# drnatebrown/col-bwt

Hardware: AMD Instinct MI355X
Metric: query bases/s (higher is better)
Workload: dtype int64

## Files before the change

col-bwt_amd/csrc/fat2_query.hip:

```cpp
#include <hip/hip_runtime.h>
#include <stdint.h>

#include "device_layout.h"
#include "fat_cursor.h"
#include "fat_layout.h"
#include "lane_io.h"
#include "lane_out.h"
#include "query_kernels.h"

namespace colbwt {

namespace {

constexpr uint32_t kOffMis0 = 0xFFFFFFFCu;
constexpr uint32_t kOffMis1 = 0xFFFFFFFBu;

#ifdef COLBWT_COUNT_TRIPS
#define FAT2_STAT(k) (++stat[k])
__device__ unsigned long long g_fat2_more[2];
#else
#define FAT2_STAT(k) ((void)0)
#endif

__device__ __forceinline__ uint32_t mis_slot(const uint8_t *top, uint32_t own, uint32_t c) {
    const uint32_t aidx = top[own], cidx = top[c];
    const uint32_t slot = cidx < aidx ? cidx : cidx - 1;
    return cidx < 4 && slot < kFatSlots ? slot : kFatSlots;
}

template <int K, typename PmlT, bool kDeep>
__global__ __launch_bounds__(kQueryBlock)
void fat2_query_kernel(FatTable T, const uint8_t *__restrict__ bases, const uint64_t *__restrict__ read_off,
                       uint64_t n_reads, uint32_t big_reads, uint32_t tail_permille,
                       PmlT *__restrict__ pml, uint8_t *__restrict__ cid) {
    constexpr bool kWide = sizeof(PmlT) == 4;
    constexpr bool kTail = K == 8 && !kWide;
    __shared__ uint4 s_stage[kWaves][8][64];
    __shared__ uint4 s_win[kWaves][4][64];
    __shared__ uint32_t s_claim;
    __shared__ uint8_t s_top[256];
    __shared__ uint32_t s_tch[kTail ? 256 : 1];
    const uint32_t wave = threadIdx.x >> 6, lane = threadIdx.x & 63u, g8 = lane & ~7u, p = lane & 7u;
    uint32_t *const s_jx = reinterpret_cast<uint32_t *>(&s_stage[wave][7][48]);
    ChunkPlan plan;
    plan.init(n_reads, big_reads, tail_permille);
    if (threadIdx.x == 0) s_claim = 0;
    s_top[threadIdx.x] = (uint8_t)fat_top_index(T.top4, threadIdx.x);
    if constexpr (kTail) {
        const uint32_t b = threadIdx.x;
        s_tch[b] = ((T.top4 >> (8 * (b & 3u))) & 0xFFu) | (((T.top4 >> (8 * ((b >> 2) & 3u))) & 0xFFu) << 8) |
                   (((T.top4 >> (8 * ((b >> 4) & 3u))) & 0xFFu) << 16) | (((T.top4 >> (8 * (b >> 6))) & 0xFFu) << 24);
    }
    __syncthreads();
    uint32_t *const claim = &s_claim;
    ReadCursor rc;
    bool done;
    rc.c_next = threadIdx.x;
    rc.request_chunk(plan, read_off);
    rc.commit();
    done = !rc.enter_chunk(plan, claim);

    OutRuns acc;
    uint32_t trip = 0;
    LaneWindow win;
    win.init(rc.off + rc.k - 1);
    uint4 (*const my_win)[64] = s_win[wave];

    uint32_t j = done ? 0u : T.r - 1;
    uint32_t o = kOffLastPos;
    uint32_t L = 0;
    const uint4 *const my_row = &s_stage[wave][p][g8];

#ifdef COLBWT_COUNT_TRIPS
    unsigned long long stat[8] = {0, 0, 0, 0, 0, 0, 0, 0}, stat_full = 0, stat_hop15 = 0;
#endif
    while (__any(!done)) {
        bool step_back = false;
        if (!done && rc.k == 0 && !rc.next_in_flight && (rc.r != rc.r_lo || rc.nc_ready)) {
            if (rc.r != rc.r_lo) {
                rc.r -= 1;
                rc.k = rc.off - rc.next_off;
                rc.off = rc.next_off;
                step_back = rc.r > rc.r_lo;
            } else if (kWide || acc.cnt == 0) {
                done = !rc.enter_chunk(plan, claim);
                if (!done) win.init(rc.off + rc.k - 1);
            }
            j = done ? 0u : T.r - 1;
            o = kOffLastPos;
            L = 0;
        }
        const bool live = !done && rc.k != 0;
        uint64_t &k = rc.k;
        const uint64_t g = rc.off + k - 1;

        s_jx[lane] = j;
        wave_sync();
        {
            const uint4 ja = *reinterpret_cast<const uint4 *>(&s_jx[g8]);
            const uint4 jb = *reinterpret_cast<const uint4 *>(&s_jx[g8 + 4]);
            const uint32_t jq[8] = {ja.x, ja.y, ja.z, ja.w, jb.x, jb.y, jb.z, jb.w};
            wave_sync();
#pragma unroll
            for (uint32_t q = 0; q < 8; ++q)
                __builtin_amdgcn_global_load_lds(T.lines + (uint64_t)jq[q] * kFatRowBytes + ((p ^ q) << 4), &s_stage[wave][q][0],
                                                 16, 0, 0);
        }
        uint32_t want = 8u;
        if constexpr (kTail) want = T.match_tail && L >= 8u && o != kOffMis0 && o != kOffMis1 ? 16u : 8u;
        if (live && win.avail(g) < (k < want ? (uint32_t)k : want)) win.request(my_win, bases, g);
        if (step_back) { rc.in_next = read_off[rc.r - 1]; rc.next_in_flight = true; }
        if (!done && rc.fetch_pending) rc.request_chunk(plan, read_off);
        lds_dma_landed();
        rc.commit();

        const uint32_t have = live ? win.avail(g) : 0u;
        uint32_t consumed = 0, l_new = 0, keep = 0xFFFFFFFFu, keep1 = 0xFFFFFFFFu;
        uint64_t ids = 0, ids2 = 0;
        if (!live || have == 0) FAT2_STAT(5);
        if (live && have != 0) {
            const uint64_t W = win.get8(my_win, lane, g);
            const uint32_t left = k < have ? (uint32_t)k : have;
            if (o == kOffMis0 || o == kOffMis1) {
                FAT2_STAT(2);
                const uint32_t h4 = !kDeep && o == kOffMis1 ? 4u : 0u;
                const uint4 e0 = my_row[(h4 + 0u) ^ p], e1 = my_row[(h4 + 1u) ^ p], e2 = my_row[(h4 + 2u) ^ p],
                            e3 = my_row[(h4 + 3u) ^ p];
                const uint32_t carry = L;
                const uint32_t t1 = (e0.y >> 16) & 0xFFu, d1 = e0.y >> 24, v1 = e3.z & 7u;
                uint32_t oc = 4;
                if (left >= 2) {
                    const uint32_t c2 = (uint32_t)(W >> 48) & 0xFFu;
                    const uint32_t s2 = mis_slot(s_top, t1, c2);
                    if (c2 == t1) oc = 0;
                    else if (s2 < kFatSlots && ((v1 >> s2) & 1u)) oc = 1 + s2;
                }
                if (oc < 4) {
                    const uint32_t J = oc == 0 ? e0.z : oc == 1 ? e0.w : oc == 2 ? e1.x : e1.y;
                    const uint32_t rho = oc == 0 ? e1.z : oc == 1 ? e1.w : oc == 2 ? e2.x : e2.y;
                    const uint32_t pw = oc < 2 ? e2.z : e2.w, P = (oc & 1u) ? pw >> 16 : pw & 0xFFFFu;
                    const uint32_t ch = (e3.x >> (8 * oc)) & 0xFFu, cd = (e3.y >> (8 * oc)) & 0xFFu;
                    const uint32_t vo = (e3.z >> (4 + 4 * oc)) & 7u;
                    consumed = 2;
                    l_new = 1;
                    keep = oc == 0 ? 0xFFFFFFFFu : 0u;
                    ids = (uint64_t)(d1 | (carry << 8));
                    L = oc == 0 ? 1u : 0u;
                    uint32_t nJ = J, nP = P, nrho = rho, nch = ch, ncd = cd, nv = vo, seen = 2;
                    if constexpr (kDeep) {
                        if (left >= 3 && ((uint32_t)(W >> 40) & 0xFFu) == ch) {
                            const uint4 f0 = my_row[4u ^ p], f1 = my_row[5u ^ p], f2 = my_row[6u ^ p], f3 = my_row[7u ^ p];
                            nJ = oc == 0 ? f0.x : oc == 1 ? f0.y : oc == 2 ? f0.z : f0.w;
                            nrho = oc == 0 ? f1.x : oc == 1 ? f1.y : oc == 2 ? f1.z : f1.w;
                            const uint32_t pw2 = oc < 2 ? f2.x : f2.y;
                            nP = (oc & 1u) ? pw2 >> 16 : pw2 & 0xFFFFu;
                            nch = (f2.z >> (8 * oc)) & 0xFFu;
                            ncd = (f2.w >> (8 * oc)) & 0xFFu;
                            nv = (f3.x >> (4 * oc)) & 7u;
                            consumed = 3;
                            seen = 3;
                            ids = (uint64_t)(cd | (d1 << 8) | (carry << 16));
                            if (oc == 0) { l_new = 2; keep = 0xFFFFFFFFu; }
                            else { l_new = 1; keep = 0xFFFFFFFFu; keep1 = 0u; }
                            L += 1;
                        }
                    }
                    if (k > consumed) {
                        uint32_t sn = kFatSlots;
                        if (left > seen) {
                            const uint32_t cn = (uint32_t)(W >> (8u * (7u - seen))) & 0xFFu;
                            if (cn != nch) sn = mis_slot(s_top, nch, cn);
                        }
                        if (sn < kFatSlots && ((nv >> sn) & 1u)) {
                            const uint32_t e = nrho * kFatSlots + sn;
                            j = T.slot_line0 + (kDeep ? e : e >> 1);
                            o = kDeep ? kOffMis0 : kOffMis0 - (e & 1u);
                            L = ncd;
                        } else {
                            j = nJ;
                            o = nP;
                        }
                    }
                } else {
                    consumed = 1;
                    l_new = 0;
                    ids = (uint64_t)carry;
                    L = 0;
                    j = e0.x;
                    o = e0.y & 0xFFFFu;
                }
            } else {
                FAT2_STAT(0);
                const uint4 r0 = my_row[0 ^ p];
                const uint4 r1 = my_row[1 ^ p];
                const uint64_t CH = (uint64_t)r0.x | ((uint64_t)r0.y << 32);
                const uint64_t CID = (uint64_t)r0.z | ((uint64_t)r0.w << 32);
                const uint32_t len = r1.x & 0xFFFFu;
                uint32_t skip = 0;
                bool stay = false;
                if (o == kOffPred) { o = len - 1; skip = 1; }
                else if (o == kOffSucc) { o = 0; skip = 1; }
                else if (o >= len && j < T.r - 1) {
                    o -= len;
                    j += 1;
                    stay = true;
                    FAT2_STAT(1);
                } else {
                    o = o < len ? o : len - 1;
                }
                if (!stay) {
                    const uint64_t X = skip ? ((W >> 8) ^ CH) & 0x00FFFFFFFFFFFFFFull : W ^ CH;
                    const uint32_t run = matching_top_bytes(X);
                    const uint32_t cap = left + skip < (uint32_t)K ? left + skip : (uint32_t)K;
                    uint32_t steps = run < cap ? run : cap;
                    bool own_jump = true, to_entry = false;
                    uint32_t e_next = 0, carry = 0;
                    bool hop = false;
                    uint4 tl = make_uint4(0u, 0u, 0u, 0u);
                    if constexpr (kTail) {
                        if (T.match_tail && run == 8u && left + skip >= 16u && o < (r1.x >> 24) &&
                            acc.cnt + 16u + 8u * (3u - (trip & 3u)) <= 96u) {
                            tl = my_row[7 ^ p];
                            const uint64_t W2 = win.get8(my_win, lane, g - (8u - skip));
                            const uint64_t TC = (uint64_t)s_tch[(tl.w >> 16) & 0xFFu] | ((uint64_t)s_tch[tl.w >> 24] << 32);
                            hop = W2 == TC;
                        }
                    }
#ifdef COLBWT_COUNT_TRIPS
                    if (K == 8 && run == 8u && cap == 8u) ++stat_full;
#endif
                    if (run < cap) {
                        const uint32_t d = run + 1u, sh = 8u * (8u - d);
                        const uint32_t c = (uint32_t)(W >> (sh + 8u * skip)) & 0xFFu;
                        const uint32_t s = mis_slot(s_top, (uint32_t)(CH >> sh) & 0xFFu, c);
                        if (s < kFatSlots && ((r1.w >> (3u * run + s)) & 1u)) {
                            const uint32_t rho = reinterpret_cast<const uint32_t *>(&my_row[((kFatRho / 16) + (run >> 2)) ^ p])[run & 3u];
                            e_next = rho * kFatSlots + s;
                            carry = (uint32_t)(CID >> sh) & 0xFFu;
                            to_entry = true;
                            own_jump = false;
                        }
                    }
                    if (run == 0 && !to_entry) {
                        const uint32_t c = (uint32_t)(W >> 56);
                        const uint32_t cidx = T.cmap[c];
                        bool moved = false;
                        if (cidx != kAbsent) moved = fat_threshold_scan(T, j, o, c, cidx);
                        FAT2_STAT(moved ? 3 : 4);
                        if (moved) {
                            steps = 1;
                            consumed = 1;
                            l_new = 0;
                            own_jump = false;
                        } else {
                            const uint32_t st = matching_top_bytes(X & 0x00FFFFFFFFFFFFFFull);
                            const uint32_t cap0 = left < (uint32_t)K ? left : (uint32_t)K;
                            steps = st < cap0 ? st : cap0;
                            consumed = steps;
                            l_new = steps - 1;
                        }
                    } else {
                        consumed = (hop ? 16u : steps) - skip;
                        l_new = L + consumed;
                    }
                    L = l_new;
                    ids = steps ? CID >> (8u * (8u - steps)) : 0ull;
                    if (hop) {
                        FAT2_STAT(7);
#ifdef COLBWT_COUNT_TRIPS
                        stat_hop15 += skip;
#endif
                        ids2 = ids;
                        ids = (uint64_t)tl.x | ((uint64_t)tl.y << 32);
                    }
                    if (k == consumed) {
                    } else if (hop) {
                        j = tl.z;
                        o += tl.w & 0xFFFFu;
                    } else if (to_entry) {
                        FAT2_STAT(6);
                        j = T.slot_line0 + (kDeep ? e_next : e_next >> 1);
                        o = kDeep ? kOffMis0 : kOffMis0 - (e_next & 1u);
                        L = carry;
                    } else if (own_jump) {
                        const uint32_t e = steps - 1;
                        const uint32_t I = reinterpret_cast<const uint32_t *>(&my_row[((kFatI / 16) + (e >> 2)) ^ p])[e & 3u];
                        const uint32_t Oh = reinterpret_cast<const uint16_t *>(&my_row[((kFatO / 16) + (e >> 3)) ^ p])[e & 7u];
                        const uint64_t cuts = (uint64_t)r1.y | ((uint64_t)r1.z << 32);
                        const uint32_t cut = (uint32_t)(cuts >> (8 * e)) & 0xFFu, cut_a = cut & 0xFu, len_b = cut >> 4;
                        j = I;
                        if (cut_a != kSKCutNone && o >= cut_a) {
                            j += 1;
                            o -= cut_a;
                            if (len_b != kSKCutNone && o >= len_b) {
                                j += 1;
                                o -= len_b;
                            }
                        } else {
                            o += Oh;
                        }
                    }
                }
            }
            if constexpr (kWide) {
                for (uint32_t e = 0; e < consumed; ++e) {
                    pml[g - consumed + 1 + e] = (PmlT)((e < 2 ? keep : keep1) ? l_new - e : 0u);
                    cid[g - consumed + 1 + e] = (uint8_t)(ids >> (8 * e));
                }
            } else {
                if constexpr (kTail) acc.template push_run<true>(consumed, l_new, keep, keep1, (uint32_t)ids, (uint32_t)(ids >> 32), (uint32_t)ids2, (uint32_t)(ids2 >> 32));
                else acc.push_run(consumed, l_new, keep, keep1, (uint32_t)ids, (uint32_t)(ids >> 32));
            }
            k -= consumed;
        }
        wave_sync();
        if constexpr (!kWide) {
#ifdef COLBWT_ABL_NO_FLUSH
            if ((trip & (OutRuns::kPeriod - 1)) == OutRuns::kPeriod - 1) acc.cnt = acc.cnt > 90 ? 1 : 0;
#else
            if ((trip & (OutRuns::kPeriod - 1)) == OutRuns::kPeriod - 1)
                acc.flush_wave((uint16_t *)pml, cid, rc.off + rc.k, !done, rc.k == 0 && rc.r == rc.r_lo, &s_stage[wave][0][0], lane);
#endif
        }
        ++trip;
        wave_sync();
    }
#ifdef COLBWT_COUNT_TRIPS
    for (int q = 0; q < 8; ++q) atomicAdd(&g_fat_stats[q], stat[q]);
    atomicAdd(&g_fat2_more[0], stat_full);
    atomicAdd(&g_fat2_more[1], stat_hop15);
#endif
}

template <int K>
void launch_steps2(const FatTable &T, const uint8_t *d_bases, const uint64_t *d_read_off, uint64_t n_reads, uint64_t n_bases,
                   void *d_pml, int pml_bytes, uint8_t *d_cid, hipStream_t stream) {
    const bool deep = T.entry_shift == 7;
    if (pml_bytes == 2 && deep) launch_persistent<fat2_query_kernel<K, uint16_t, true>>(T, d_bases, d_read_off, n_reads, n_bases, (uint16_t *)d_pml, d_cid, stream);
    else if (pml_bytes == 2) launch_persistent<fat2_query_kernel<K, uint16_t, false>>(T, d_bases, d_read_off, n_reads, n_bases, (uint16_t *)d_pml, d_cid, stream);
    else if (deep) launch_persistent<fat2_query_kernel<K, uint32_t, true>>(T, d_bases, d_read_off, n_reads, n_bases, (uint32_t *)d_pml, d_cid, stream);
    else launch_persistent<fat2_query_kernel<K, uint32_t, false>>(T, d_bases, d_read_off, n_reads, n_bases, (uint32_t *)d_pml, d_cid, stream);
}

}

void launch_fat2_query(const FatTable &T, const uint8_t *d_bases, const uint64_t *d_read_off, uint64_t n_reads, uint64_t n_bases,
                       void *d_pml, int pml_bytes, uint8_t *d_cid, hipStream_t stream) {
    if (n_reads == 0) return;
#define X(K) \
    if (T.steps == K) launch_steps2<K>(T, d_bases, d_read_off, n_reads, n_bases, d_pml, pml_bytes, d_cid, stream);
    COLBWT_FAT_STEPS(X)
#undef X
}

#ifdef COLBWT_COUNT_TRIPS
extern "C" int colbwt_debug_fat2_stats(unsigned long long *out10, int reset) {
    if (hipMemcpyFromSymbol(out10, HIP_SYMBOL(g_fat_stats), 8 * sizeof(unsigned long long)) != hipSuccess) return -1;
    if (hipMemcpyFromSymbol(out10 + 8, HIP_SYMBOL(g_fat2_more), 2 * sizeof(unsigned long long)) != hipSuccess) return -1;
    if (reset) {
        unsigned long long z[8] = {0, 0, 0, 0, 0, 0, 0, 0};
        if (hipMemcpyToSymbol(HIP_SYMBOL(g_fat_stats), z, sizeof(z)) != hipSuccess) return -1;
        if (hipMemcpyToSymbol(HIP_SYMBOL(g_fat2_more), z, 2 * sizeof(unsigned long long)) != hipSuccess) return -1;
    }
    return 0;
}
#endif

}
```

col-bwt_amd/csrc/fat_build.hip:

```cpp
#include <hip/hip_runtime.h>
#include <stdint.h>

#include <functional>
#include <string>
#include <vector>

#include "../../include/colbwt.h"
#include "dev_mem.h"
#include "device_layout.h"
#include "fat_layout.h"
#include "jump_tables.h"
#include "lf_device.h"
#include "query_kernels.h"
#include "read_sampler.h"
#include "refine.h"

namespace colbwt {

namespace {

struct PlainLevel {
    const uint64_t *idx;
    const uint32_t *I;
    const uint16_t *O;
// ... 218 lines not shown
        }
        put_byte(w, kFatCut + (s - 1), cut | (len_b << 4));
    }

    if constexpr (kMis && K == 8) {
        uint64_t span = len < kFatTSpanMax ? len : kFatTSpanMax;
        uint32_t tch = 0;
        for (uint32_t a = 1; a <= kFatTailSteps + 1; ++a) {
            const uint64_t jl = P.idx[(uint64_t)j + 1] - P.idx[j];
            const uint64_t room = t < jl ? jl - t : 0;
            span = span < room ? span : room;
            if (a > kFatTailSteps) break;
            const uint32_t meta = P.meta[j];
            const uint32_t x = fat_top_index(T.top4, meta & 0xFFu);
            if (x >= 4) span = 0;
            tch |= (x & 3u) << (2 * (8 - a));
            put_byte(w, kFatTCid + (8 - a), meta >> 8);
            plain_lf(P, j, t);
        }
        if (span != 0) {
            put_half(w, kFatTCh, tch);
            w[kFatTI / 4] = j;
            put_half(w, kFatTO, (uint32_t)t);
            put_byte(w, kFatTSpan, (uint32_t)span);
            atomicAdd(tail_rows, 1ull);
        } else {
            w[kFatTCid / 4] = 0;
            w[kFatTCid / 4 + 1] = 0;
        }
    }
    if constexpr (kMis) {
        put_byte(w, kFatFlags, sflags[i]);
    } else {
        const uint32_t a_dense = T.cmap[own_ch];
        const uint32_t aidx = a_dense < 4 ? a_dense : kFatOwnOther;
        uint32_t flags = aidx << 4;
        const uint32_t top = T.sigma < 4 ? T.sigma : 4;
        for (uint32_t cidx = 0; cidx < top; ++cidx) {
            if (cidx == a_dense) continue;
            const uint32_t slot = hint_slot(cidx, a_dense);
            if (slot >= kFatSlots) continue;
            uint32_t tj;
            uint64_t to;
            if (!fat_slot_target(P, T, i, cidx, tj, to)) continue;
            flags |= 1u << slot;
            const uint32_t sb = kFatSlot0 + slot * kFatSlotBytes;
            plain_lf(P, tj, to);
            w[sb >> 2] = tj;
            put_half(w, sb + kFatSlotP, (uint32_t)to);
            const uint32_t meta = P.meta[tj];
            put_byte(w, sb + kFatSlotCh2, meta & 0xFFu);
            put_byte(w, sb + kFatSlotCid2, meta >> 8);
            plain_lf(P, tj, to);
            w[(sb >> 2) + 1] = tj;
            put_half(w, sb + kFatSlotP + 2, (uint32_t)to);
        }
        put_byte(w, kFatFlags, flags);
    }
    uint4 *dst = reinterpret_cast<uint4 *>(lines + (uint64_t)i * kFatRowBytes);
#pragma unroll
    for (uint32_t q = 0; q < kFatRowBytes / 16; ++q) dst[q] = make_uint4(w[4 * q], w[4 * q + 1], w[4 * q + 2], w[4 * q + 3]);
}

template <bool kDeep>
__global__ __launch_bounds__(256) void fat_mis_pack_kernel(PlainLevel P, FatTable T, const uint32_t *__restrict__ rho,
                                                           const uint32_t *__restrict__ rho_first,
                                                           const uint8_t *__restrict__ sflags, uint8_t *__restrict__ entries) {
    const uint64_t e = (uint64_t)blockIdx.x * 256 + threadIdx.x;
    if (e >= (uint64_t)T.n_rho * kFatSlots) return;
    constexpr uint32_t kDwords = (kDeep ? 2 * kMisBytes : kMisBytes) / 4;
    uint32_t w[kDwords];
#pragma unroll
    for (uint32_t q = 0; q < kDwords; ++q) w[q] = 0;
    const uint32_t i = rho_first[e / kFatSlots], slot = (uint32_t)(e % kFatSlots);
    if ((sflags[i] >> slot) & 1u) {
        const uint32_t a_dense = T.cmap[P.meta[i] & 0xFFu];
        uint32_t tj;
        uint64_t to;
        fat_slot_target(P, T, i, slot < a_dense ? slot : slot + 1, tj, to);
        plain_lf(P, tj, to);
        const uint32_t J1 = tj;
        const uint64_t P1 = to;
        const uint32_t m1 = P.meta[J1], a1 = T.cmap[m1 & 0xFFu], v1 = sflags[J1] & 7u;
        w[kMisJ1] = J1;
        w[kMisP1] = (uint32_t)P1 | ((m1 & 0xFFu) << 16) | ((m1 >> 8) << 24);
        w[kMisVal] = v1;
        for (uint32_t o = 0; o < 4; ++o) {
            uint32_t j = J1;
            uint64_t t = P1;
            if (o) {
                if (!((v1 >> (o - 1)) & 1u)) continue;
                fat_slot_target(P, T, J1, (o - 1) < a1 ? o - 1 : o, j, t);
            }
            plain_lf(P, j, t);
            const uint32_t m = P.meta[j];
            w[kMisJ + o] = j;
            w[kMisRho + o] = rho[j];
            put_half(w, 4 * kMisP + 2 * o, (uint32_t)t);
            put_byte(w, 4 * kMisCh + o, m & 0xFFu);
            put_byte(w, 4 * kMisCid + o, m >> 8);
            w[kMisVal] |= (uint32_t)(sflags[j] & 7u) << (4 + 4 * o);
            if constexpr (kDeep) {
                plain_lf(P, j, t);
                const uint32_t m2 = P.meta[j];
                w[kMisDeep + kMisJ - 2 + o] = j;
                w[kMisDeep + kMisRho - 2 + o] = rho[j];
                put_half(w, 4 * (kMisDeep + kMisP - 2) + 2 * o, (uint32_t)t);
                put_byte(w, 4 * (kMisDeep + kMisCh - 2) + o, m2 & 0xFFu);
                put_byte(w, 4 * (kMisDeep + kMisCid - 2) + o, m2 >> 8);
                w[kMisDeep + kMisVal - 2] |= (uint32_t)(sflags[j] & 7u) << (4 * o);
            }
        }
    }
    uint4 *dst = reinterpret_cast<uint4 *>(entries + e * (kDwords * 4));
#pragma unroll
    for (uint32_t q = 0; q < kDwords / 4; ++q) dst[q] = make_uint4(w[4 * q], w[4 * q + 1], w[4 * q + 2], w[4 * q + 3]);
}

template <class Src>
int refine_plain(const Src &S, uint64_t src_rows, uint64_t n, PlainLevel &out, PlainBuffers &buf, std::string &err) {
    DevPtr first, park;
    uint64_t total = 0;
    {
        const int rc = count_and_scan(S, src_rows, first, total, err);
        if (rc != COLBWT_OK) return rc;
    }
    if (total > 0xFFFFFFFEull) {
        err = "line-row layout needs " + std::to_string(total) + " rows at one of its levels (> 2^32-2)";
        return COLBWT_ERR_NOMEM;
    }
    if (total * kFatRowBytes > dev_available_bytes()) {
        if (getenv("COLBWT_ALLOC_LOG"))
            fprintf(stderr, "[colbwt alloc] ? %llu rows x 128 bytes = %.2f GB against %.2f GB available\n", (unsigned long long)total,
                    total * 128e-9, dev_available_bytes() * 1e-9);
        err = "line-row layout: " + std::to_string(total) + " rows at a refinement level need more HBM than is available";
        return COLBWT_ERR_NOMEM;
    }
    const uint32_t r_new = (uint32_t)total;
    SK_TRY(buf.idx.alloc(((uint64_t)r_new + 2) * sizeof(uint64_t)));
    SK_TRY(buf.I.alloc(((uint64_t)r_new + 1) * sizeof(uint32_t)));
    SK_TRY(buf.O.alloc(((uint64_t)r_new + 1) * sizeof(uint16_t)));
    SK_TRY(buf.meta.alloc(((uint64_t)r_new + 1) * sizeof(uint16_t)));
    SK_TRY(buf.thr.alloc(((uint64_t)r_new + 1) * sizeof(uint64_t)));
    SK_TRY(buf.org.alloc((uint64_t)r_new + 1));
    SK_TRY(park.alloc(((uint64_t)r_new + 1) * sizeof(uint64_t)));
    uint64_t *const d_idx = buf.idx.as<uint64_t>(), *const d_thr = buf.thr.as<uint64_t>(), *const d_park = park.as<uint64_t>();
    uint32_t *const d_I = buf.I.as<uint32_t>(), *const d_first = first.as<uint32_t>();
    uint16_t *const d_O = buf.O.as<uint16_t>(), *const d_meta = buf.meta.as<uint16_t>();
    uint8_t *const d_org = buf.org.as<uint8_t>();
    const uint32_t rblocks = (uint32_t)((src_rows + 255) / 256);
    hipLaunchKernelGGL(plain_emit_kernel<Src>, dim3(rblocks), dim3(256), 0, 0, S, (const uint32_t *)d_first, d_idx, d_I, d_meta,
                       d_thr, d_org, d_park, r_new);
    SK_TRY(hipGetLastError());
    SK_TRY(hipStreamSynchronize(0));
    const uint32_t nblocks = (uint32_t)(((uint64_t)r_new + 255) / 256);
    hipLaunchKernelGGL(plain_link_kernel, dim3(nblocks), dim3(256), 0, 0, (const uint32_t *)d_first, (const uint64_t *)d_idx,
                       (const uint64_t *)d_park, d_I, d_O, r_new);
    SK_TRY(hipGetLastError());
    SK_TRY(hipStreamSynchronize(0));
    out.idx = d_idx;
    out.I = d_I;
    out.O = d_O;
    out.meta = d_meta;
    out.thr = d_thr;
    out.org = d_org;
    out.n = n;
    out.r = r_new;
    return COLBWT_OK;
}

constexpr uint64_t kDeepReserve = 32ull << 30;

template <int K>
int build_fat_steps(const DevTable &T1, const HintChars &chars, int mismatch_lines, FatTable &out, FatBuffers &buf, std::string &err,
                    const std::function<void()> &source_done, int &failed_level) {
    failed_level = 2;
    const uint8_t *cmap = T1.cmap;
    const uint32_t sigma = T1.sigma;
    PlainLevel cur{};
    PlainBuffers cur_buf;
    LoadClock clock;
    {
        const SrcL1 s1{T1, chars};
        const int rc = refine_plain(s1, T1.r, T1.n, cur, cur_buf, err);
        if (rc != COLBWT_OK) return rc;
    }
    clock.lap("  refinement level 2");
    source_done();
    clock.lap("  one-step tables freed");
    for (int level = 3; level <= K; ++level) {
        failed_level = level;
        PlainLevel next{};
        PlainBuffers next_buf;
// ... 210 lines not shown
```

col-bwt_amd/csrc/fat_layout.h:

```cpp
#pragma once
#include <hip/hip_runtime.h>
#include <stdint.h>

#include "device_layout.h"

namespace colbwt {

#define COLBWT_FAT_STEPS(X) X(4) X(5) X(6) X(7) X(8)

constexpr uint32_t kFatRowBytes = 128;
constexpr uint32_t kFatSlots = 3;
constexpr uint32_t kFatSlotSteps = 2;
constexpr uint32_t kFatOwnOther = 7;
constexpr uint32_t kFatCh = 0, kFatCid = 8, kFatLen = 16, kFatFlags = 18, kFatCut = 20, kFatI = 32, kFatO = 64,
                   kFatSlot0 = 80, kFatSlotBytes = 16;
constexpr uint32_t kFatSlotP = 8, kFatSlotCh2 = 12, kFatSlotCid2 = 13;
constexpr uint32_t kFatVal = 28, kFatRho = 80;
constexpr uint32_t kFatTSpan = 19, kFatTCid = 112, kFatTI = 120, kFatTO = 124, kFatTCh = 126;
constexpr uint32_t kFatTailSteps = 8, kFatTSpanMax = 255;
constexpr uint32_t kMisBytes = 64, kMisJ1 = 0, kMisP1 = 1, kMisJ = 2, kMisRho = 6, kMisP = 10, kMisCh = 12, kMisCid = 13, kMisVal = 14;
constexpr uint32_t kMisDeep = 16;

struct FatTable {
    const uint8_t *lines;
    const uint8_t *chr;
    const uint64_t *idx;
    const uint64_t *thr;
    const uint32_t *next_tbl;
    const uint32_t *prev_tbl;
    const uint8_t *cmap;
    uint64_t n;
    uint32_t r;
    uint32_t sigma;
    uint32_t nblk;
    uint32_t steps;
    uint32_t top4;
    uint32_t slot_line0;
    uint32_t n_rho;
    uint32_t entry_shift;
    uint32_t match_tail;
    uint32_t tail_permille;
};

__device__ __forceinline__ uint32_t fat_byte(const uint32_t *w, uint32_t off) { return (w[off >> 2] >> (8 * (off & 3u))) & 0xFFu; }
__device__ __forceinline__ uint32_t fat_half(const uint32_t *w, uint32_t off) { return (w[off >> 2] >> (8 * (off & 2u))) & 0xFFFFu; }

__device__ __forceinline__ uint32_t fat_top_index(uint32_t top4, uint32_t c) {
    uint32_t x = 4;
    x = ((top4 >> 24) & 0xFFu) == c ? 3u : x;
    x = ((top4 >> 16) & 0xFFu) == c ? 2u : x;
    x = ((top4 >> 8) & 0xFFu) == c ? 1u : x;
    x = (top4 & 0xFFu) == c ? 0u : x;
    return x;
}

__device__ __forceinline__ uint32_t fat_succ_char(const FatTable &T, uint32_t i, uint32_t c, uint32_t cidx) {
    const uint32_t blk = i >> kBlockShift;
    const uint64_t lim = (((uint64_t)blk + 1) << kBlockShift);
    const uint64_t end = lim < T.r ? lim : T.r;
    for (uint64_t s = (uint64_t)i + 1; s < end; ++s)
        if (T.chr[s] == c) return (uint32_t)s;
    if (blk + 1 < T.nblk) return T.next_tbl[(uint64_t)(blk + 1) * T.sigma + cidx];
    return kNone;
}
__device__ __forceinline__ uint32_t fat_pred_char(const FatTable &T, uint32_t i, uint32_t c, uint32_t cidx) {
    const uint32_t blk = i >> kBlockShift;
    const uint32_t first = blk << kBlockShift;
    for (uint32_t q = i; q > first;) {
        --q;
        if (T.chr[q] == c) return q;
    }
    if (blk > 0) return T.prev_tbl[(uint64_t)blk * T.sigma + cidx];
    return kNone;
}

}
```

col-bwt_amd/csrc/lane_out.h:

```cpp
#pragma once
#include <hip/hip_runtime.h>
#include <stdint.h>

#include "lane_io.h"

#ifdef COLBWT_ABL_NO_STORES
#define COLBWT_ABL_IF if (ltop == 0xFFFFFFF1u)
#else
#define COLBWT_ABL_IF
#endif

namespace colbwt {

struct OutRuns {
    static constexpr uint32_t kBlock = 64;
    static constexpr uint32_t kPeriod = 4;
    static constexpr uint32_t kSlotQ = 6, kItemQ = 4;
    static constexpr uint32_t lds_q(uint32_t slots) { return slots * kSlotQ + 2 * slots * kItemQ; }

    uint32_t z0a = 0, z0b = 0, z0c = 0, z1a = 0, z1b = 0, z1c = 0;
    uint32_t ltop = 0;
    uint32_t c0 = 0, c1 = 0, c2 = 0, c3 = 0, c4 = 0, c5 = 0, c6 = 0, c7 = 0, c8 = 0, c9 = 0, c10 = 0, c11 = 0, c12 = 0, c13 = 0, c14 = 0, c15 = 0, c16 = 0, c17 = 0, c18 = 0, c19 = 0, c20 = 0, c21 = 0, c22 = 0, c23 = 0;
    uint32_t cnt = 0;

    template <bool kUpTo16 = false>
    __device__ __forceinline__ void push_run(uint32_t n, uint32_t l_new, uint32_t keep, uint32_t keep1, uint32_t ids_lo,
                                             uint32_t ids_hi, uint32_t ids2_lo = 0, uint32_t ids2_hi = 0) {
        const uint32_t in_run = (1u << n) - 1u;
        uint32_t p0 = l_new < n ? 1u << l_new : 0u;
        p0 |= (keep ? 0u : 3u) & in_run;
        p0 |= (keep1 ? 0u : 0xCu) & in_run;
        const uint32_t top = (1u << n) >> 1;
        const uint32_t p1 = (keep & keep1) != 0u && l_new == n ? top : 0u;
        z0c = (uint32_t)(((((uint64_t)z0c << 32) | z0b) << n) >> 32);
        z0b = (uint32_t)(((((uint64_t)z0b << 32) | z0a) << n) >> 32);
        z0a = (z0a << n) | p0;
        z1c = (uint32_t)(((((uint64_t)z1c << 32) | z1b) << n) >> 32);
        z1b = (uint32_t)(((((uint64_t)z1b << 32) | z1a) << n) >> 32);
        z1a = (z1a << n) | p1;
        if constexpr (kUpTo16) {
            const bool d8 = n & 16u;
            c23 = d8 ? c19 : c23;
            c22 = d8 ? c18 : c22;
            c21 = d8 ? c17 : c21;
            c20 = d8 ? c16 : c20;
            c19 = d8 ? c15 : c19;
            c18 = d8 ? c14 : c18;
            c17 = d8 ? c13 : c17;
            c16 = d8 ? c12 : c16;
            c15 = d8 ? c11 : c15;
            c14 = d8 ? c10 : c14;
            c13 = d8 ? c9 : c13;
            c12 = d8 ? c8 : c12;
            c11 = d8 ? c7 : c11;
            c10 = d8 ? c6 : c10;
            c9 = d8 ? c5 : c9;
            c8 = d8 ? c4 : c8;
            c7 = d8 ? c3 : c7;
            c6 = d8 ? c2 : c6;
            c5 = d8 ? c1 : c5;
            c4 = d8 ? c0 : c4;
            c3 = d8 ? 0u : c3;
            c2 = d8 ? 0u : c2;
            c1 = d8 ? 0u : c1;
            c0 = d8 ? 0u : c0;
        }
        const bool d4 = n & 8u, d2 = n & 4u;
        c23 = d4 ? c21 : c23;
        c22 = d4 ? c20 : c22;
        c21 = d4 ? c19 : c21;
        c20 = d4 ? c18 : c20;
        c19 = d4 ? c17 : c19;
        c18 = d4 ? c16 : c18;
        c17 = d4 ? c15 : c17;
        c16 = d4 ? c14 : c16;
        c15 = d4 ? c13 : c15;
        c14 = d4 ? c12 : c14;
        c13 = d4 ? c11 : c13;
        c12 = d4 ? c10 : c12;
        c11 = d4 ? c9 : c11;
        c10 = d4 ? c8 : c10;
        c9 = d4 ? c7 : c9;
        c8 = d4 ? c6 : c8;
        c7 = d4 ? c5 : c7;
        c6 = d4 ? c4 : c6;
        c5 = d4 ? c3 : c5;
        c4 = d4 ? c2 : c4;
        c3 = d4 ? c1 : c3;
        c2 = d4 ? c0 : c2;
        c1 = d4 ? 0u : c1;
        c0 = d4 ? 0u : c0;
        c23 = d2 ? c22 : c23;
        c22 = d2 ? c21 : c22;
        c21 = d2 ? c20 : c21;
        c20 = d2 ? c19 : c20;
        c19 = d2 ? c18 : c19;
        c18 = d2 ? c17 : c18;
        c17 = d2 ? c16 : c17;
        c16 = d2 ? c15 : c16;
        c15 = d2 ? c14 : c15;
        c14 = d2 ? c13 : c14;
        c13 = d2 ? c12 : c13;
        c12 = d2 ? c11 : c12;
        c11 = d2 ? c10 : c11;
        c10 = d2 ? c9 : c10;
        c9 = d2 ? c8 : c9;
        c8 = d2 ? c7 : c8;
        c7 = d2 ? c6 : c7;
        c6 = d2 ? c5 : c6;
        c5 = d2 ? c4 : c5;
        c4 = d2 ? c3 : c4;
        c3 = d2 ? c2 : c3;
        c2 = d2 ? c1 : c2;
        c1 = d2 ? c0 : c1;
        c0 = d2 ? 0u : c0;
        const uint32_t sel8 = 0x07060504u - 0x01010101u * (n & 3u);
        c23 = __builtin_amdgcn_perm(c23, c22, sel8);
        c22 = __builtin_amdgcn_perm(c22, c21, sel8);
        c21 = __builtin_amdgcn_perm(c21, c20, sel8);
        c20 = __builtin_amdgcn_perm(c20, c19, sel8);
        c19 = __builtin_amdgcn_perm(c19, c18, sel8);
        c18 = __builtin_amdgcn_perm(c18, c17, sel8);
        c17 = __builtin_amdgcn_perm(c17, c16, sel8);
        c16 = __builtin_amdgcn_perm(c16, c15, sel8);
        c15 = __builtin_amdgcn_perm(c15, c14, sel8);
        c14 = __builtin_amdgcn_perm(c14, c13, sel8);
        c13 = __builtin_amdgcn_perm(c13, c12, sel8);
        c12 = __builtin_amdgcn_perm(c12, c11, sel8);
        c11 = __builtin_amdgcn_perm(c11, c10, sel8);
        c10 = __builtin_amdgcn_perm(c10, c9, sel8);
        c9 = __builtin_amdgcn_perm(c9, c8, sel8);
        c8 = __builtin_amdgcn_perm(c8, c7, sel8);
        c7 = __builtin_amdgcn_perm(c7, c6, sel8);
        c6 = __builtin_amdgcn_perm(c6, c5, sel8);
        c5 = __builtin_amdgcn_perm(c5, c4, sel8);
        c4 = __builtin_amdgcn_perm(c4, c3, sel8);
        c3 = __builtin_amdgcn_perm(c3, c2, sel8);
        c2 = __builtin_amdgcn_perm(c2, c1, sel8);
        c1 = __builtin_amdgcn_perm(c1, c0, sel8);
        c0 = __builtin_amdgcn_perm(c0, 0u, sel8);
        const uint32_t mlo = n >= 4 ? 0xFFFFFFFFu : (1u << (8 * n)) - 1u;
        const uint32_t mhi = n >= 8 ? 0xFFFFFFFFu : (n > 4 ? (1u << (8 * (n - 4))) - 1u : 0u);
        c0 |= ids_lo & mlo;
        c1 |= ids_hi & mhi;
        if constexpr (kUpTo16) {
            const uint32_t m2 = n >= 12 ? 0xFFFFFFFFu : (n > 8 ? (1u << (8 * (n - 8))) - 1u : 0u);
            const uint32_t m3 = n >= 16 ? 0xFFFFFFFFu : (n > 12 ? (1u << (8 * (n - 12))) - 1u : 0u);
            c2 |= ids2_lo & m2;
            c3 |= ids2_hi & m3;
        }
        cnt += n;
    }

    static __device__ __forceinline__ void shr96(uint64_t &lo, uint32_t &hi, uint32_t s) {
        if (s >= 64) {
            lo = (uint64_t)(hi >> (s - 64));
            hi = 0;
        } else if (s) {
            lo = (lo >> s) | ((uint64_t)hi << (64 - s));
            hi = s < 32 ? hi >> s : 0u;
        }
    }
    static __device__ __forceinline__ uint64_t low64_from(uint32_t a, uint32_t b, uint32_t c, uint32_t s) {
        uint64_t lo = ((uint64_t)b << 32) | a;
        uint32_t hi = c;
        shr96(lo, hi, s);
        return lo;
    }
    __device__ __forceinline__ uint32_t park_item(uint4 *item, uint32_t slot, uint32_t e_lo, uint32_t count, uint64_t addr, uint32_t lt) const {
        const uint32_t o_lo = (uint32_t)addr & (kBlock - 1), o_hi = o_lo + count;
        const uint64_t in_item = count >= 64 ? ~0ull : (1ull << count) - 1ull;
        const uint64_t Z0 = (low64_from(z0a, z0b, z0c, e_lo) & in_item) << o_lo;
        const uint64_t Z1 = (low64_from(z1a, z1b, z1c, e_lo) & in_item) << o_lo;
        const uint32_t z0w[2] = {(uint32_t)Z0, (uint32_t)(Z0 >> 32)}, z1w[2] = {(uint32_t)Z1, (uint32_t)(Z1 >> 32)};
        uint32_t pm[8];
        uint32_t v = lt;
#pragma unroll
        for (int p = 7; p >= 0; --p) {
            const uint32_t b0 = (z0w[p >> 2] >> (8 * (p & 3))) & 0xFFu, b1 = (z1w[p >> 2] >> (8 * (p & 3))) & 0xFFu;
            pm[p] = (v & 0xFFFFu) | (b0 << 16) | (b1 << 24);
            const uint32_t lo_p = o_lo > 8u * p ? o_lo : 8u * p, hi_p = o_hi < 8u * p + 8u ? o_hi : 8u * p + 8u;
            if (hi_p > lo_p) {
                const uint32_t bits = b0 | b1;
                if (bits) {
                    const uint32_t q = (uint32_t)__builtin_ctz(bits);
                    v = q - (lo_p - 8u * p) + ((b1 >> q) & 1u);
                } else {
                    v += hi_p - lo_p;
                }
            }
        }
        item[0] = make_uint4(slot, e_lo, count, (uint32_t)addr);
        item[1] = make_uint4((uint32_t)(addr >> 32), 0u, 0u, 0u);
        item[2] = make_uint4(pm[0], pm[1], pm[2], pm[3]);
        item[3] = make_uint4(pm[4], pm[5], pm[6], pm[7]);
        return v;
    }

    template <uint32_t kSlots = 32>
    __device__ __forceinline__ void flush_wave(uint16_t *pml, uint8_t *cid, uint64_t gl, bool active, bool final, uint4 *lds,
                                               uint32_t lane) {
        constexpr uint32_t kItemBase = kSlots * kSlotQ;
        const uint32_t below = (0u - (uint32_t)gl) & (kBlock - 1);
        const bool has_a = active && below < cnt;
        const uint32_t rest = below < cnt ? below : cnt;
        const bool has_b = active && final && rest != 0;
        const unsigned long long emit = __ballot(has_a || has_b);
        if (emit == 0) return;
        const uint32_t n_a = has_a ? cnt - below : 0u;
        uint32_t v_cut = ltop;
        const unsigned long long lt = (1ull << lane) - 1ull;
        const uint32_t rank = (uint32_t)__builtin_popcountll(emit & lt), lanes = (uint32_t)__builtin_popcountll(emit);
        for (uint32_t first = 0; first < lanes; first += kSlots) {
            const bool mine = (has_a || has_b) && rank >= first && rank < first + kSlots;
            const bool rag_a = mine && has_a && n_a != kBlock, rag_b = mine && has_b, full_a = mine && has_a && n_a == kBlock;
            const unsigned long long m_ra = __ballot(rag_a), m_rb = __ballot(rag_b), m_fa = __ballot(full_a);
            const uint32_t n_ra = (uint32_t)__builtin_popcountll(m_ra), n_rb = (uint32_t)__builtin_popcountll(m_rb);
            const uint32_t n_rag = n_ra + n_rb, n_items = n_rag + (uint32_t)__builtin_popcountll(m_fa);
            if (mine) {
                uint4 *slot = lds + kSlotQ * (rank - first);
                slot[0] = make_uint4(c0, c1, c2, c3);
                slot[1] = make_uint4(c4, c5, c6, c7);
                slot[2] = make_uint4(c8, c9, c10, c11);
// ... 105 lines not shown
```

Measured before the change: 146.8 billion.

## Repack deep mismatch lines per outcome and precompute top indices

```diff
diff --git a/col-bwt_amd/csrc/fat2_query.hip b/col-bwt_amd/csrc/fat2_query.hip
--- a/col-bwt_amd/csrc/fat2_query.hip
+++ b/col-bwt_amd/csrc/fat2_query.hip
@@ -17,16 +17,19 @@
 
 #ifdef COLBWT_COUNT_TRIPS
 #define FAT2_STAT(k) (++stat[k])
+__device__ unsigned long long g_fat2_oc[9];
+#define FAT2_OC(k) (++stat_oc[k])
 __device__ unsigned long long g_fat2_more[2];
 #else
 #define FAT2_STAT(k) ((void)0)
-#endif
-
-__device__ __forceinline__ uint32_t mis_slot(const uint8_t *top, uint32_t own, uint32_t c) {
-    const uint32_t aidx = top[own], cidx = top[c];
+#define FAT2_OC(k) ((void)0)
+#endif
+
+__device__ __forceinline__ uint32_t mis_slot_at(uint32_t aidx, uint32_t cidx) {
     const uint32_t slot = cidx < aidx ? cidx : cidx - 1;
     return cidx < 4 && slot < kFatSlots ? slot : kFatSlots;
 }
+__device__ __forceinline__ uint32_t mis_slot(const uint8_t *top, uint32_t own, uint32_t c) { return mis_slot_at(top[own], top[c]); }
 
 template <int K, typename PmlT, bool kDeep>
 __global__ __launch_bounds__(kQueryBlock)
@@ -73,6 +76,7 @@
 
 #ifdef COLBWT_COUNT_TRIPS
     unsigned long long stat[8] = {0, 0, 0, 0, 0, 0, 0, 0}, stat_full = 0, stat_hop15 = 0;
+    unsigned long long stat_oc[9] = {0, 0, 0, 0, 0, 0, 0, 0, 0};
 #endif
     while (__any(!done)) {
         bool step_back = false;
@@ -124,23 +128,39 @@
             if (o == kOffMis0 || o == kOffMis1) {
                 FAT2_STAT(2);
                 const uint32_t h4 = !kDeep && o == kOffMis1 ? 4u : 0u;
-                const uint4 e0 = my_row[(h4 + 0u) ^ p], e1 = my_row[(h4 + 1u) ^ p], e2 = my_row[(h4 + 2u) ^ p],
-                            e3 = my_row[(h4 + 3u) ^ p];
+                uint4 e0, e1, e2, e3;
                 const uint32_t carry = L;
-                const uint32_t t1 = (e0.y >> 16) & 0xFFu, d1 = e0.y >> 24, v1 = e3.z & 7u;
+                uint32_t t1, d1, v1, a1;
+                if constexpr (kDeep) {
+                    const uint32_t hd = reinterpret_cast<const uint32_t *>(&my_row[kMisDeepHdr ^ p])[kMisDeepAux];
+                    t1 = hd & 0xFFu, d1 = (hd >> kMisDeepHdrD1) & 0xFFu, v1 = (hd >> kMisDeepHdrV1) & 7u, a1 = (hd >> kMisDeepHdrTop) & 7u;
+                } else {
+                    e0 = my_row[(h4 + 0u) ^ p], e1 = my_row[(h4 + 1u) ^ p], e2 = my_row[(h4 + 2u) ^ p], e3 = my_row[(h4 + 3u) ^ p];
+                    t1 = (e0.y >> 16) & 0xFFu, d1 = e0.y >> 24, v1 = e3.z & 7u, a1 = s_top[t1];
+                }
                 uint32_t oc = 4;
                 if (left >= 2) {
                     const uint32_t c2 = (uint32_t)(W >> 48) & 0xFFu;
-                    const uint32_t s2 = mis_slot(s_top, t1, c2);
+                    const uint32_t s2 = mis_slot_at(a1, s_top[c2]);
                     if (c2 == t1) oc = 0;
                     else if (s2 < kFatSlots && ((v1 >> s2) & 1u)) oc = 1 + s2;
                 }
                 if (oc < 4) {
-                    const uint32_t J = oc == 0 ? e0.z : oc == 1 ? e0.w : oc == 2 ? e1.x : e1.y;
-                    const uint32_t rho = oc == 0 ? e1.z : oc == 1 ? e1.w : oc == 2 ? e2.x : e2.y;
-                    const uint32_t pw = oc < 2 ? e2.z : e2.w, P = (oc & 1u) ? pw >> 16 : pw & 0xFFFFu;
-                    const uint32_t ch = (e3.x >> (8 * oc)) & 0xFFu, cd = (e3.y >> (8 * oc)) & 0xFFu;
-                    const uint32_t vo = (e3.z >> (4 + 4 * oc)) & 7u;
+                    uint32_t J, rho, P, ch, cd, vo;
+                    uint32_t ntop = 0;
+                    uint4 ea;
+                    if constexpr (kDeep) {
+                        ea = my_row[oc ^ p];
+                        J = ea.x, rho = ea.y, P = ea.z & 0xFFFFu, ch = (ea.z >> 16) & 0xFFu, cd = ea.z >> 24;
+                        vo = (ea.w >> kMisDeepV) & 7u, ntop = (ea.w >> kMisDeepTop) & 7u;
+                    } else {
+                        J = oc == 0 ? e0.z : oc == 1 ? e0.w : oc == 2 ? e1.x : e1.y;
+                        rho = oc == 0 ? e1.z : oc == 1 ? e1.w : oc == 2 ? e2.x : e2.y;
+                        const uint32_t pw = oc < 2 ? e2.z : e2.w;
+                        P = (oc & 1u) ? pw >> 16 : pw & 0xFFFFu;
+                        ch = (e3.x >> (8 * oc)) & 0xFFu, cd = (e3.y >> (8 * oc)) & 0xFFu;
+                        vo = (e3.z >> (4 + 4 * oc)) & 7u;
+                    }
                     consumed = 2;
                     l_new = 1;
                     keep = oc == 0 ? 0xFFFFFFFFu : 0u;
@@ -149,14 +169,9 @@
                     uint32_t nJ = J, nP = P, nrho = rho, nch = ch, ncd = cd, nv = vo, seen = 2;
                     if constexpr (kDeep) {
                         if (left >= 3 && ((uint32_t)(W >> 40) & 0xFFu) == ch) {
-                            const uint4 f0 = my_row[4u ^ p], f1 = my_row[5u ^ p], f2 = my_row[6u ^ p], f3 = my_row[7u ^ p];
-                            nJ = oc == 0 ? f0.x : oc == 1 ? f0.y : oc == 2 ? f0.z : f0.w;
-                            nrho = oc == 0 ? f1.x : oc == 1 ? f1.y : oc == 2 ? f1.z : f1.w;
-                            const uint32_t pw2 = oc < 2 ? f2.x : f2.y;
-                            nP = (oc & 1u) ? pw2 >> 16 : pw2 & 0xFFFFu;
-                            nch = (f2.z >> (8 * oc)) & 0xFFu;
-                            ncd = (f2.w >> (8 * oc)) & 0xFFu;
-                            nv = (f3.x >> (4 * oc)) & 7u;
+                            const uint4 eb = my_row[(kMisDeepStep3 + oc) ^ p];
+                            nJ = eb.x, nrho = eb.y, nP = eb.z & 0xFFFFu, nch = (eb.z >> 16) & 0xFFu, ncd = eb.z >> 24;
+                            nv = (ea.w >> kMisDeepV3) & 7u, ntop = (ea.w >> kMisDeepTop3) & 7u;
                             consumed = 3;
                             seen = 3;
                             ids = (uint64_t)(cd | (d1 << 8) | (carry << 16));
@@ -165,11 +180,12 @@
                             L += 1;
                         }
                     }
+                    FAT2_OC(2u * oc + (consumed == 3u ? 1u : 0u));
                     if (k > consumed) {
                         uint32_t sn = kFatSlots;
                         if (left > seen) {
                             const uint32_t cn = (uint32_t)(W >> (8u * (7u - seen))) & 0xFFu;
-                            if (cn != nch) sn = mis_slot(s_top, nch, cn);
+                            if (cn != nch) sn = mis_slot_at(kDeep ? ntop : (uint32_t)s_top[nch], s_top[cn]);
                         }
                         if (sn < kFatSlots && ((nv >> sn) & 1u)) {
                             const uint32_t e = nrho * kFatSlots + sn;
@@ -182,12 +198,18 @@
                         }
                     }
                 } else {
+                    FAT2_OC(8);
                     consumed = 1;
                     l_new = 0;
                     ids = (uint64_t)carry;
                     L = 0;
-                    j = e0.x;
-                    o = e0.y & 0xFFFFu;
+                    if constexpr (kDeep) {
+                        j = reinterpret_cast<const uint32_t *>(&my_row[kMisDeepHdrJ1 ^ p])[kMisDeepAux];
+                        o = reinterpret_cast<const uint32_t *>(&my_row[kMisDeepHdrP1 ^ p])[kMisDeepAux] & 0xFFFFu;
+                    } else {
+                        j = e0.x;
+                        o = e0.y & 0xFFFFu;
+                    }
                 }
             } else {
                 FAT2_STAT(0);
@@ -327,6 +349,7 @@
     }
 #ifdef COLBWT_COUNT_TRIPS
     for (int q = 0; q < 8; ++q) atomicAdd(&g_fat_stats[q], stat[q]);
+    for (int q = 0; q < 9; ++q) atomicAdd(&g_fat2_oc[q], stat_oc[q]);
     atomicAdd(&g_fat2_more[0], stat_full);
     atomicAdd(&g_fat2_more[1], stat_hop15);
 #endif
@@ -364,6 +387,14 @@
     }
     return 0;
 }
-#endif
-
-}
+extern "C" int colbwt_debug_fat2_outcomes(unsigned long long *out9, int reset) {
+    if (hipMemcpyFromSymbol(out9, HIP_SYMBOL(g_fat2_oc), 9 * sizeof(unsigned long long)) != hipSuccess) return -1;
+    if (reset) {
+        unsigned long long z[9] = {0, 0, 0, 0, 0, 0, 0, 0, 0};
+        if (hipMemcpyToSymbol(HIP_SYMBOL(g_fat2_oc), z, sizeof(z)) != hipSuccess) return -1;
+    }
+    return 0;
+}
+#endif
+
+}
diff --git a/col-bwt_amd/csrc/fat_build.hip b/col-bwt_amd/csrc/fat_build.hip
--- a/col-bwt_amd/csrc/fat_build.hip
+++ b/col-bwt_amd/csrc/fat_build.hip
@@ -324,9 +324,16 @@
         const uint32_t J1 = tj;
         const uint64_t P1 = to;
         const uint32_t m1 = P.meta[J1], a1 = T.cmap[m1 & 0xFFu], v1 = sflags[J1] & 7u;
-        w[kMisJ1] = J1;
-        w[kMisP1] = (uint32_t)P1 | ((m1 & 0xFFu) << 16) | ((m1 >> 8) << 24);
-        w[kMisVal] = v1;
+        if constexpr (kDeep) {
+            w[4 * kMisDeepHdrJ1 + kMisDeepAux] = J1;
+            w[4 * kMisDeepHdrP1 + kMisDeepAux] = (uint32_t)P1;
+            w[4 * kMisDeepHdr + kMisDeepAux] = (m1 & 0xFFu) | ((m1 >> 8) << kMisDeepHdrD1) | (v1 << kMisDeepHdrV1) |
+                                               (fat_top_index(T.top4, m1 & 0xFFu) << kMisDeepHdrTop);
+        } else {
+            w[kMisJ1] = J1;
+            w[kMisP1] = (uint32_t)P1 | ((m1 & 0xFFu) << 16) | ((m1 >> 8) << 24);
+            w[kMisVal] = v1;
+        }
         for (uint32_t o = 0; o < 4; ++o) {
             uint32_t j = J1;
             uint64_t t = P1;
@@ -336,21 +343,25 @@
             }
             plain_lf(P, j, t);
             const uint32_t m = P.meta[j];
-            w[kMisJ + o] = j;
-            w[kMisRho + o] = rho[j];
-            put_half(w, 4 * kMisP + 2 * o, (uint32_t)t);
-            put_byte(w, 4 * kMisCh + o, m & 0xFFu);
-            put_byte(w, 4 * kMisCid + o, m >> 8);
-            w[kMisVal] |= (uint32_t)(sflags[j] & 7u) << (4 + 4 * o);
             if constexpr (kDeep) {
+                uint32_t *const a = w + 4 * o, *const b = w + 4 * (kMisDeepStep3 + o);
+                a[kMisDeepJ] = j;
+                a[kMisDeepRho] = rho[j];
+                a[kMisDeepPcc] = ((uint32_t)t & 0xFFFFu) | ((m & 0xFFu) << 16) | ((m >> 8) << 24);
+                a[kMisDeepAux] |= ((uint32_t)(sflags[j] & 7u) << kMisDeepV) | (fat_top_index(T.top4, m & 0xFFu) << kMisDeepTop);
                 plain_lf(P, j, t);
                 const uint32_t m2 = P.meta[j];
-                w[kMisDeep + kMisJ - 2 + o] = j;
-                w[kMisDeep + kMisRho - 2 + o] = rho[j];
-                put_half(w, 4 * (kMisDeep + kMisP - 2) + 2 * o, (uint32_t)t);
-                put_byte(w, 4 * (kMisDeep + kMisCh - 2) + o, m2 & 0xFFu);
-                put_byte(w, 4 * (kMisDeep + kMisCid - 2) + o, m2 >> 8);
-                w[kMisDeep + kMisVal - 2] |= (uint32_t)(sflags[j] & 7u) << (4 * o);
+                b[kMisDeepJ] = j;
+                b[kMisDeepRho] = rho[j];
+                b[kMisDeepPcc] = ((uint32_t)t & 0xFFFFu) | ((m2 & 0xFFu) << 16) | ((m2 >> 8) << 24);
+                a[kMisDeepAux] |= ((uint32_t)(sflags[j] & 7u) << kMisDeepV3) | (fat_top_index(T.top4, m2 & 0xFFu) << kMisDeepTop3);
+            } else {
+                w[kMisJ + o] = j;
+                w[kMisRho + o] = rho[j];
+                put_half(w, 4 * kMisP + 2 * o, (uint32_t)t);
+                put_byte(w, 4 * kMisCh + o, m & 0xFFu);
+                put_byte(w, 4 * kMisCid + o, m >> 8);
+                w[kMisVal] |= (uint32_t)(sflags[j] & 7u) << (4 + 4 * o);
             }
         }
     }
diff --git a/col-bwt_amd/csrc/fat_layout.h b/col-bwt_amd/csrc/fat_layout.h
--- a/col-bwt_amd/csrc/fat_layout.h
+++ b/col-bwt_amd/csrc/fat_layout.h
@@ -19,7 +19,11 @@
 constexpr uint32_t kFatTSpan = 19, kFatTCid = 112, kFatTI = 120, kFatTO = 124, kFatTCh = 126;
 constexpr uint32_t kFatTailSteps = 8, kFatTSpanMax = 255;
 constexpr uint32_t kMisBytes = 64, kMisJ1 = 0, kMisP1 = 1, kMisJ = 2, kMisRho = 6, kMisP = 10, kMisCh = 12, kMisCid = 13, kMisVal = 14;
-constexpr uint32_t kMisDeep = 16;
+constexpr uint32_t kMisDeepJ = 0, kMisDeepRho = 1, kMisDeepPcc = 2, kMisDeepAux = 3;
+constexpr uint32_t kMisDeepStep3 = 4;
+constexpr uint32_t kMisDeepV = 0, kMisDeepTop = 4, kMisDeepV3 = 8, kMisDeepTop3 = 12;
+constexpr uint32_t kMisDeepHdrJ1 = 4, kMisDeepHdrP1 = 5, kMisDeepHdr = 6;
+constexpr uint32_t kMisDeepHdrD1 = 8, kMisDeepHdrV1 = 16, kMisDeepHdrTop = 20;
 
 struct FatTable {
     const uint8_t *lines;
diff --git a/col-bwt_amd/csrc/lane_out.h b/col-bwt_amd/csrc/lane_out.h
--- a/col-bwt_amd/csrc/lane_out.h
+++ b/col-bwt_amd/csrc/lane_out.h
@@ -38,6 +38,7 @@
         z1c = (uint32_t)(((((uint64_t)z1c << 32) | z1b) << n) >> 32);
         z1b = (uint32_t)(((((uint64_t)z1b << 32) | z1a) << n) >> 32);
         z1a = (z1a << n) | p1;
+#ifndef COLBWT_ABL_NO_IDNET
         if constexpr (kUpTo16) {
             const bool d8 = n & 16u;
             c23 = d8 ? c19 : c23;
@@ -139,6 +140,7 @@
         c2 = __builtin_amdgcn_perm(c2, c1, sel8);
         c1 = __builtin_amdgcn_perm(c1, c0, sel8);
         c0 = __builtin_amdgcn_perm(c0, 0u, sel8);
+#endif
         const uint32_t mlo = n >= 4 ? 0xFFFFFFFFu : (1u << (8 * n)) - 1u;
         const uint32_t mhi = n >= 8 ? 0xFFFFFFFFu : (n > 4 ? (1u << (8 * (n - 4))) - 1u : 0u);
         c0 |= ids_lo & mlo;
```

Result: no change. 147.2 billion, median of 6 (+0.3%).
